# crstnbr/detqmc

Hardware: AMD Instinct MI355X
Metric: DQMC sweeps/sec (SDW-O2 L=16 beta=10 fp64) (higher is better)
Workload: dtype f64; 1 GPU; DetSDW O(2) L=16 beta=10 dtau=0.1 s=10 checkerboard delayed(32) sweepThermalization, 512 independent chains per GPU (1 process x 4 kernel contexts x 128 lockstep chains), stabilisation=qr; n_g=512, m=100, replicas_per_gpu=512, processes_per_gpu=1, contexts_per_process=4, chains_per_context=128, launch=self

## Files before the change

detqmc_amd/csrc/dqmc_context.hip:

```cpp
#include "dqmc_ctx.h"
#include <cmath>
#include <complex>
#include <cstddef>
#include <cstdio>
#include <cstdlib>
#include <cstring>
#include <string>
#include <vector>

void build_tournament(int nblk, std::vector<int>& out);

thread_local std::string g_err;

template<class T>
static int dalloc(dqmc_ctx* c, T** p, size_t count) {
    const size_t bytes = (count * sizeof(T) + 255) & ~(size_t)255;
    *p = (T*)(uintptr_t)(c->arena_off + 256);
    c->fixups.push_back((void**)p);
    c->arena_off += bytes;
    return 0;
}
static int arena_commit(dqmc_ctx* c) {
    const size_t cs = c->arena_off;
    void* q = nullptr;
// ... 242 lines not shown
            for (int y = 0; y < L; ++y)
                for (int x = 0; x < L; ++x) {
                    const int coord = dirn == 0 ? x : y;
                    if ((coord & 1) != parity) continue;
                    const int a = y * L + x, b = neigh[(dirn == 0 ? 0 : 2) * N + a];
                    M[(size_t)a * N + b] += shv; M[(size_t)b * N + a] += shv;
                }
            return M;
        };
        auto mul = [&](const std::vector<double>& A, const std::vector<double>& B) {
            std::vector<double> C((size_t)N * N, 0.0);
            for (int i = 0; i < N; ++i) for (int k = 0; k < N; ++k) { const double a = A[(size_t)i * N + k]; if (a != 0.0) for (int j = 0; j < N; ++j) C[(size_t)i * N + j] += a * B[(size_t)k * N + j]; }
            return C;
        };
        const std::vector<double> F = mul(mul(bond_matrix(0, 0, sh), bond_matrix(0, 1, sh)), mul(bond_matrix(1, 0, sh), bond_matrix(1, 1, sh)));
        const std::vector<double> Fi = mul(mul(bond_matrix(1, 1, -sh), bond_matrix(1, 0, -sh)), mul(bond_matrix(0, 1, -sh), bond_matrix(0, 0, -sh)));
        Em.assign((size_t)N * N, hc(0.0)); Ep.assign((size_t)N * N, hc(0.0));
        for (size_t i = 0; i < (size_t)N * N; ++i) { Em[i] = F[i]; Ep[i] = Fi[i]; }
    }
    out_minus.assign((size_t)ng * ng, hc(0.0)); out_plus.assign((size_t)ng * ng, hc(0.0));
    for (int b = 0; b < 2; ++b)
        for (int i = 0; i < N; ++i) for (int j = 0; j < N; ++j) {
            out_minus[(size_t)(b * N + j) * ng + (b * N + i)] = Em[(size_t)i * N + j];
            out_plus[(size_t)(b * N + j) * ng + (b * N + i)] = Ep[(size_t)i * N + j];
        }
}

static int alloc_qr_work(dqmc_ctx* c) {
    const int ng = c->n_g, np = (ng + 15) / 16;
    const size_t n2 = (size_t)ng * ng;
    int rc;
#define A_(x) if ((rc = (x))) return rc;
    A_(dalloc(c, &c->qw.V, n2)); A_(dalloc(c, &c->qw.T, (size_t)np * 2 * 256));
    A_(dalloc(c, &c->qw.W, (size_t)16 * ng)); A_(dalloc(c, &c->qw.W2, (size_t)16 * ng)); A_(dalloc(c, &c->qw.Rneg, (size_t)32 * ng));
    if (ng > 1024) { c->qw.part_count = (size_t)ng * 64 * 8; A_(dalloc(c, &c->qw.part, c->qw.part_count)); }
    A_(dalloc(c, &c->qr_perm, (size_t)ng)); A_(dalloc(c, &c->lu_swaps, (size_t)LU_SWAP_INTS)); A_(dalloc(c, &c->lu_tneg, (size_t)ng * 32)); A_(dalloc(c, &c->qr_perm_inv, (size_t)ng)); A_(dalloc(c, &c->qr_dinv, (size_t)ng));
    A_(dalloc(c, &c->rmax_inv, (size_t)ng)); A_(dalloc(c, &c->rmin, (size_t)ng));
    A_(dalloc(c, &c->lmax_inv, (size_t)ng)); A_(dalloc(c, &c->lmin, (size_t)ng));
#undef A_
    return 0;
}

static int alloc_slot(dqmc_ctx* c, UdVSlot& sl) {
    size_t n2 = (size_t)c->n_g * c->n_g;
    int rc;
    if ((rc = dalloc(c, &sl.U, n2))) return rc;
    if ((rc = dalloc(c, &sl.d, (size_t)c->n_g))) return rc;
    if ((rc = dalloc(c, &sl.Vt, n2))) return rc;
    return 0;
}

extern "C" int dqmc_create(const dqmc_params* p, dqmc_ctx** out) { return dqmc_create_batch(p, 1, out); }
static int create_fill(dqmc_ctx* c, const dqmc_params* p);

extern "C" int dqmc_create_batch(const dqmc_params* p, int nchains, dqmc_ctx** out) {
    if (!p || !out) return fail(DQMC_EINVAL, "null argument");
    *out = nullptr;
    if (nchains < 1 || nchains > 1024) return fail(DQMC_EINVAL, "nchains must be in 1..1024");
    if (p->opdim < 1 || p->opdim > 3) return fail(DQMC_EINVAL, "opdim must be 1, 2 or 3");
    if (p->L < 2 || (p->L % 2) != 0)
        return fail(DQMC_EINVAL, "Checker board decomposition only supported for even linear lattice sizes");
    if (p->weakZflux && p->opdim != 2) return fail(DQMC_EINVAL, "Magnetic field currently only supported for opdim=2");
    if (p->m < 2 || p->s < 1 || p->s >= p->m) return fail(DQMC_EINVAL, "need 0 < s < m");
    const int N = p->L * p->L, MSF = p->opdim == 3 ? 4 : 2;
    if (p->delaySteps < 1 || p->delaySteps > N) return fail(DQMC_EINVAL, "delaySteps must be in 1..N");
    if (MSF * p->delaySteps > DQMC_MAX_WDIM) return fail(DQMC_EINVAL, "MSF*delaySteps must be <= 64 on this build");
// ... 1405 lines not shown
```

detqmc_amd/csrc/dqmc_internal.h:

```cpp
#pragma once
#include <hip/hip_runtime.h>
#include <stdint.h>
#include "../../include/dqmc_hip.h"

#include <stdlib.h>
#include <float.h>
static inline const char* dev_knob(const char* name) {
#ifdef DQMC_DEV_KNOBS
    return getenv(name);
#else
    (void)name;
    return nullptr;
#endif
}

typedef double2 cplx;

#define DQMC_MAX_MSF 4
#define DQMC_MAX_WDIM 64
#define DQMC_DECIDE_WIDE_MAX_CHAINS 32

enum { SUBFAM_LU_UPDATE = 0, SUBFAM_FACT_GEMM = 1, SUBFAM_COUNT = 4 };
struct SubProf { void (*begin)(void* user, int sub); void (*end)(void* user, int sub, double flops, double bytes); void* user; };
struct Launch { hipStream_t st; int nb; size_t cs; const SubProf* sub = nullptr; };
// ... 247 lines not shown
size_t measure_custom_bond_table_cplx(int count, int N);
void launch_td_custom_onebody(const Launch& lc, const DevModel& hm, int count, const cplx* M, const unsigned* mask, const cplx* gs, cplx* ob, int t,
                              const CustomBond* bond = nullptr);
void launch_measure_td_custom(const Launch& lc, const DevModel& hm, int count, const cplx* M, const unsigned* mask, const cplx* gs, const cplx* hs,
                              const cplx* ob, double* acc, size_t acs, int row, int rows, const CustomBond* bond = nullptr);
void launch_measure_eq_custom(const Launch& lc, const DevModel& hm, int count, const cplx* M, const unsigned* mask, const cplx* M2, const unsigned* mask2,
                              const cplx* gs, cplx* ob, double* acc, const CustomBond* bond = nullptr);
struct CustomPair { const cplx* tab; const unsigned* mk; unsigned parts[DQMC_CUSTOM_MAX]; };
size_t measure_custom_pair_table_cplx(int count, int N);
void launch_measure_custom_pair(const Launch& lc, const DevModel& hm, int count, const cplx* Fa, const unsigned* mask, const cplx* gs, double* acc,
                                size_t acs, int row, int rows, const CustomPair* pair = nullptr);
size_t measure_green_matrix_row_doubles(int opdim, int N);
void launch_measure_green_matrix(const Launch& lc, const DevModel& hm, const cplx* gs, double* acc, size_t acs, int row, int rows, int apbx, int apby);
void launch_series_green_sample(const Launch& lc, const DevModel& hm, const double* fine, size_t chain_bytes, double* sample, size_t S, size_t off,
                                double* bad);
size_t series_pair_bubble_lds_bytes(int opdim, int N);
bool launch_series_pair_vertex(const Launch& lc, const DevModel& hm, const double* bins, const double* mean, const double* trig, size_t S, int B,
                               int nfreq, size_t off_chi, size_t off_g, int count, const CustomPair& pair, int qx, int qy, int apbx, int apby,
                               double* pb, double* value, double* err);
size_t series_ph_bubble_lds_bytes(int opdim, int N);
bool launch_series_ph_vertex(const Launch& lc, const DevModel& hm, const double* bins, const double* mean, const double* trig, size_t S, int B,
                             int nfreq, size_t off_chi, size_t off_g, int count, const CustomBond& bond, int qx, int qy, int apbx, int apby,
                             double* pb, double* value, double* err);
struct GreenCheckFold { double* table; size_t table_stride; int row; const double* d; const double* sv; };
size_t green_diff_partial_doubles(int n);
void launch_green_keep(const Launch& lc, const cplx* G, cplx* keep, size_t keep_stride, size_t count);
void launch_green_diff(const Launch& lc, const cplx* Gw, size_t gw_stride, const cplx* Gf, int n, int ld, int N, double* part,
                       size_t part_stride, double* out, size_t out_stride, const GreenCheckFold* fold = nullptr);
size_t measure_custom_row_doubles(int count, int N);
size_t measure_td_custom_onebody_cplx(int count, int N);
size_t measure_eq_custom_onebody_cplx(int count, int N);

struct SvdProfHooks;
struct QrWork { cplx* V; cplx* T; cplx* W; cplx* W2; cplx* Rneg; const SvdProfHooks* apply_hooks; cplx* part; size_t part_count; int* err; };
int run_qr(const Launch& lc, int n, cplx* A, cplx* Q, const QrWork& w);
int run_qr_apply_q(const Launch& lc, int n, cplx* C, const QrWork& w, int trans);
int run_qr_bgs(const Launch& lc, int n, cplx* A, cplx* Q, const QrWork& w);
void qr_reset_workspace(const Launch& lc, int n, const QrWork& w);
int run_trsm_right_upper(const Launch& lc, int n, const cplx* R, cplx* C, const QrWork& w, int trans = 0, int unit = 0,
                         const ColSrc* src = nullptr);
#define LU_SWAP_INTS 128
int run_lu(const Launch& lc, int n, cplx* A, int* perm, int* swaps, cplx* tneg);
void launch_gather_scale_cols(const Launch& lc, const cplx* X, const double* cs, const int* perm, int n, cplx* Y);
void launch_udt_init(const Launch& lc, const cplx* M, int ldm, const double* cs, const double* rs, const int* perm,
                     int transpose, cplx* W, int n);
void launch_udt_diag(const Launch& lc, const cplx* R, int n, double* d);
void launch_udt_lazy(const Launch& lc, const double* d, const int* perm, int n, double* dinv, int* perm_inv);
void launch_udt_tmat(const Launch& lc, const cplx* R, const double* d, const int* perm, int n, cplx* Tt);
void launch_permute_scale_cols(const Launch& lc, const cplx* X, const double* cs, const int* perm, int n, cplx* Y);
void launch_split_scales(const Launch& lc, const double* d, int n, double* dmax_inv, double* dmin);
void launch_logdet_vector(const Launch& lc, const cplx* R, const double* a, const double* b, int n, double* sv);
void launch_scaled_norms_rank(const Launch& lc, const cplx* M, int ldm, const double* cs, const double* rs, int transpose,
                              int n, double* norms, int* rank, double* scratch_d);
```

detqmc_amd/csrc/kernels_qr.hip:

```cpp
#include "dqmc_internal.h"
#include <cstring>

#define QR_NB 16

template<int CTRL, int ROWMASK>
__device__ __forceinline__ double q_dpp_add(double v) {
    int lo = __double2loint(v), hi = __double2hiint(v);
    int lo2 = __builtin_amdgcn_update_dpp(0, lo, CTRL, ROWMASK, 0xf, false);
    int hi2 = __builtin_amdgcn_update_dpp(0, hi, CTRL, ROWMASK, 0xf, false);
    return v + __hiloint2double(hi2, lo2);
}
__device__ __forceinline__ double q_readlane_d(double x, int l) {
    int lo = __builtin_amdgcn_readlane(__double2loint(x), l);
    int hi = __builtin_amdgcn_readlane(__double2hiint(x), l);
    return __hiloint2double(hi, lo);
}
__device__ __forceinline__ double q_wave_total(double v) {
    v = q_dpp_add<0xB1, 0xf>(v);
    v = q_dpp_add<0x4E, 0xf>(v);
    v = q_dpp_add<0x114, 0xf>(v);
    v = q_dpp_add<0x118, 0xf>(v);
    v = q_dpp_add<0x142, 0xa>(v);
    v = q_dpp_add<0x143, 0xc>(v);
    return q_readlane_d(v, 63);
}

template<int H, int MASK>
__device__ __forceinline__ void q_butterfly_level(double (&val)[32], int lane) {
    const bool hi = (lane & MASK) != 0;
#pragma unroll
    for (int j = 0; j < H; ++j) {
        double keep = hi ? val[j + H] : val[j];
        double send = hi ? val[j] : val[j + H];
        val[j] = keep + __shfl_xor(send, MASK, 64);
    }
}
// ... 112 lines not shown
                    cplx t = q_cmul(tv, w[c]);
                    a[r][c].x -= t.x;
                    a[r][c].y -= t.y;
                }
            }
        }
        if (tid < QR_NB) {
            int i = tid;
            cplx t = make_double2(0.0, 0.0);
            if (i < C) {
                cplx acc = make_double2(0.0, 0.0);
#pragma unroll
                for (int k = 0; k < QR_NB; ++k) {
                    if (k < C && k >= i) {
                        cplx tik = sT[k * QR_NB + i];
                        cplx t2 = q_cmul(tik, w[k]);
                        acc.x += t2.x; acc.y += t2.y;
                    }
                }
                cplx t3 = q_cmul(tau, acc);
                t = make_double2(-t3.x, -t3.y);
            } else if (i == C) {
                t = tau;
            }
            sT[C * QR_NB + i] = t;
            if (i == C) { sTau[C] = tau; sBeta[C] = beta; }
        }
        __syncthreads();
    }
};

template<int RPT, int NT>
__global__ __launch_bounds__(NT) void k_qr_panel(cplx* __restrict__ A, int lda, int n, int j0,
                                                  cplx* __restrict__ Vp, cplx* __restrict__ Tp, cplx* __restrict__ Tn, size_t cs) {
    __shared__ double red[2][NT / 64][2 * QR_NB];
    CHAIN(A); CHAIN(Vp); CHAIN(Tp); CHAIN(Tn);
    __shared__ cplx sT[QR_NB * QR_NB];
    __shared__ cplx sTau[QR_NB];
    __shared__ double sBeta[QR_NB];
    __shared__ cplx sAlpha;
    QrPanelState<RPT, NT> s;
    s.red = red; s.sT = sT; s.sTau = sTau; s.sBeta = sBeta; s.sAlpha = &sAlpha;
    s.tid = threadIdx.x; s.lane = threadIdx.x & 63; s.wave = threadIdx.x >> 6;
    s.rows = n - j0;
    s.ncols = (n - j0 < QR_NB) ? (n - j0) : QR_NB;
    for (int i = threadIdx.x; i < QR_NB * QR_NB; i += NT) sT[i] = make_double2(0.0, 0.0);
#pragma unroll
    for (int r = 0; r < RPT; ++r) {
        int row = s.tid + r * NT;
#pragma unroll
        for (int c = 0; c < QR_NB; ++c) {
            const cplx t = A[(size_t)(j0 + min(c, s.ncols - 1)) * lda + (j0 + min(row, s.rows - 1))];
            s.a[r][c] = (row < s.rows && c < s.ncols) ? t : make_double2(0.0, 0.0);
        }
    }
    __syncthreads();
    QrPanelStep<0>::run(s);
#pragma unroll
    for (int r = 0; r < RPT; ++r) {
        int row = s.tid + r * NT;
        if (row < s.rows) {
#pragma unroll
            for (int c = 0; c < QR_NB; ++c) {
                if (c >= s.ncols) continue;
                size_t off = (size_t)(j0 + c) * lda + (j0 + row);
                cplx x = s.a[r][c];
                if (row < c) {
                    A[off] = x;
                    Vp[off] = make_double2(0.0, 0.0);
                } else if (row == c) {
                    A[off] = make_double2(sBeta[c], 0.0);
                    Vp[off] = make_double2(1.0, 0.0);
                } else {
                    A[off] = make_double2(0.0, 0.0);
                    Vp[off] = x;
                }
            }
        }
    }
    for (int i = threadIdx.x; i < QR_NB * QR_NB; i += NT) {
        cplx t = sT[i];
        Tp[i] = t;
        Tn[i] = make_double2(-t.x, -t.y);
    }
}


typedef double q_v4d __attribute__((ext_vector_type(4)));
template<bool TRANS_T>
__global__ __launch_bounds__(256, 2) void k_qr_apply(const cplx* __restrict__ Vp, int ldv, const cplx* __restrict__ Tn,
                                                   cplx* __restrict__ C, int ldc, int rows, int ncols, int nb, size_t cs) {
    __shared__ cplx sV[64][QR_NB + 1];
    __shared__ cplx sC[64][QR_NB + 1];
    __shared__ cplx sW[QR_NB][QR_NB + 1];
    __shared__ cplx sT[QR_NB][QR_NB + 1];
    __shared__ cplx sPart[4][QR_NB][QR_NB + 1];
    CHAIN(Vp); CHAIN(Tn); CHAIN(C);
    const int tid = threadIdx.x, lane = tid & 63, wave = tid >> 6;
    const int l15 = lane & 15, l4 = lane >> 4;
    const int c0 = blockIdx.x * QR_NB;
    const int nc = min(QR_NB, ncols - c0);
    {
        int i = tid & 15, k = tid >> 4;
        sT[i][k] = (i < nb && k < nb) ? Tn[k * QR_NB + i] : make_double2(0.0, 0.0);
    }
    q_v4d w_re = (q_v4d)(0.0), w_im = (q_v4d)(0.0);
    for (int r0 = 0; r0 < rows; r0 += 64) {
        __syncthreads();
        for (int idx = tid; idx < 64 * QR_NB; idx += 256) {
            int rr = idx & 63, cc = idx >> 6;
            int row = r0 + rr;
// ... 40 lines not shown
#pragma unroll
    for (int ks = 0; ks < 4; ++ks) w2[ks] = sW[ks * 4 + l4][l15];
    for (int row0 = wave * 16; row0 < rows; row0 += 64) {
        const int row = row0 + l15;
        const bool rok = row < rows;
        cplx vf[4], cv[4];
#pragma unroll
        for (int ks = 0; ks < 4; ++ks) {
            const int k = ks * 4 + l4;
            const cplx tv = Vp[(size_t)min(k, nb - 1) * ldv + min(row, rows - 1)];
            vf[ks] = (rok && k < nb) ? tv : make_double2(0.0, 0.0);
        }
#pragma unroll
        for (int r = 0; r < 4; ++r) {
            const int j = l4 + 4 * r;
            cv[r] = C[(size_t)(c0 + min(j, nc - 1)) * ldc + min(row, rows - 1)];
        }
        q_v4d d_re = (q_v4d)(0.0), d_im = (q_v4d)(0.0);
#pragma unroll
        for (int ks = 0; ks < 4; ++ks) {
            d_re = __builtin_amdgcn_mfma_f64_16x16x4f64(w2[ks].x, vf[ks].x, d_re, 0, 0, 0);
            d_re = __builtin_amdgcn_mfma_f64_16x16x4f64(-w2[ks].y, vf[ks].y, d_re, 0, 0, 0);
            d_im = __builtin_amdgcn_mfma_f64_16x16x4f64(w2[ks].x, vf[ks].y, d_im, 0, 0, 0);
            d_im = __builtin_amdgcn_mfma_f64_16x16x4f64(w2[ks].y, vf[ks].x, d_im, 0, 0, 0);
        }
#pragma unroll
        for (int r = 0; r < 4; ++r) {
            const int j = l4 + 4 * r;
            if (rok && j < nc) C[(size_t)(c0 + j) * ldc + row] = make_double2(cv[r].x + d_re[r], cv[r].y + d_im[r]);
        }
    }
}

#define QR_MAXREF 4
#define QR_FENCE() do { asm volatile("" ::: "memory"); __builtin_amdgcn_sched_barrier(0); } while (0)
#define QR_TIE(acc, ptr) asm volatile("" : "+v"(acc), "+v"(ptr))
struct QrRefs { const cplx* V[QR_MAXREF]; const cplx* Tn[QR_MAXREF]; int nb[QR_MAXREF]; int n; };
template<bool TRANS_T, int NCH>
__global__ __launch_bounds__(256, 2) void k_qr_apply_reg(QrRefs refs, int ldv, cplx* __restrict__ C, int ldc, int rows, int ncols, size_t cs, int nb_chains) {
    __shared__ cplx sW[QR_NB][QR_NB + 1];
    __shared__ cplx sT[QR_NB][QR_NB + 1];
    __shared__ cplx sPart[4][QR_NB][QR_NB + 1];
    int chain, cblk;
    xcd_chain_tile((ncols + QR_NB - 1) / QR_NB, nb_chains, chain, cblk);
    C = chain_ptr_i(C, cs, chain);
    constexpr int RW = 16 * NCH;
    constexpr int NE = 4 * NCH;
    const int tid = threadIdx.x, lane = tid & 63, wave = tid >> 6;
    const int l15 = lane & 15, l4 = lane >> 4;
    const int c0 = cblk * QR_NB;
    const int nc = min(QR_NB, ncols - c0);
    const int slab = wave * RW;
    const int rlast = rows - 1;
    const bool cok = l15 < nc;
    cplx* Ccol = C + (size_t)(c0 + (cok ? l15 : 0)) * ldc;
    cplx creg[NE];
#pragma unroll
    for (int e = 0; e < NE; ++e) {
        const int row = slab + 4 * e + l4;
        const cplx t = nt_load(Ccol + min(row, rlast));
        creg[e] = (cok && row < rows) ? t : make_double2(0.0, 0.0);
    }
    const int wi = tid & 15, wj = tid >> 4;
    for (int rf = 0; rf < refs.n; ++rf) {
#if defined(__HIP_DEVICE_COMPILE__)
        typedef const cplx __attribute__((address_space(1)))* gcplx;
#else
        typedef const cplx* gcplx;
#endif
        gcplx Vp = (gcplx)chain_ptr_i(refs.V[rf], cs, chain);
        gcplx Tn = (gcplx)chain_ptr_i(refs.Tn[rf], cs, chain);
        const int nb = refs.nb[rf];
        int rl = rlast, rw = rows;
        asm volatile("" : "+v"(rl), "+s"(rw));
        __syncthreads();
        {
            const cplx t = Tn[wj * QR_NB + wi];
            sT[wi][wj] = (wi < nb && wj < nb) ? t : make_double2(0.0, 0.0);
        }
        const bool vok = l15 < nb;
        gcplx Vcol = Vp + (size_t)(vok ? l15 : 0) * ldv;
        q_v4d w_re = (q_v4d)(0.0), w_im = (q_v4d)(0.0), w_p2 = (q_v4d)(0.0);
        constexpr int CH = 4;
        cplx va[CH], vb[CH];
        auto loadv = [&](gcplx base, int e0, cplx (&dst)[CH]) {
            int rb = slab + l4;
            asm volatile("" : "+v"(rb));
#pragma unroll
            for (int i = 0; i < CH; ++i) {
                if (e0 + i >= NE) continue;
                const int row = rb + 4 * (e0 + i);
                dst[i] = base[min(row, rl)];
            }
        };
        auto mac = [&](int e0, const cplx (&src)[CH]) {
#pragma unroll
            for (int i = 0; i < CH; ++i) {
                if (e0 + i >= NE) continue;
                const cplx v = src[i];
                const cplx x = creg[e0 + i];
                w_re = __builtin_amdgcn_mfma_f64_16x16x4f64(v.x, x.x, w_re, 0, 0, 0);
                w_p2 = __builtin_amdgcn_mfma_f64_16x16x4f64(-v.y, x.y, w_p2, 0, 0, 0);
                w_im = __builtin_amdgcn_mfma_f64_16x16x4f64(v.x - v.y, x.x + x.y, w_im, 0, 0, 0);
            }
        };
        gcplx vbase = Vcol;
        loadv(vbase, 0, va);
        if (CH < NE) loadv(vbase, CH, vb);
        __builtin_amdgcn_sched_barrier(0);
#pragma unroll
        for (int c = 0; c < NE; c += 2 * CH) {
            mac(c, va);
            __builtin_amdgcn_sched_barrier(0);
            if (c + 2 * CH < NE) { QR_TIE(w_re, vbase); loadv(vbase, c + 2 * CH, va); __builtin_amdgcn_sched_barrier(0); }
            if (c + CH < NE) { mac(c + CH, vb); __builtin_amdgcn_sched_barrier(0); }
            if (c + 3 * CH < NE) { QR_TIE(w_re, vbase); loadv(vbase, c + 3 * CH, vb); __builtin_amdgcn_sched_barrier(0); }
        }
#pragma unroll
        for (int r = 0; r < 4; ++r) sPart[wave][l4 + 4 * r][l15] = make_double2(w_re[r] - w_p2[r], (w_im[r] - w_re[r]) - w_p2[r]);
        __syncthreads();
        {
            cplx p0 = sPart[0][wi][wj], p1 = sPart[1][wi][wj], p2 = sPart[2][wi][wj], p3 = sPart[3][wi][wj];
            sW[wi][wj] = make_double2((p0.x + p1.x) + (p2.x + p3.x), (p0.y + p1.y) + (p2.y + p3.y));
        }
        __syncthreads();
        {
            cplx a2 = make_double2(0.0, 0.0);
#pragma unroll
            for (int k = 0; k < QR_NB; ++k) {
                cplx t = TRANS_T ? make_double2(sT[k][wi].x, -sT[k][wi].y) : sT[wi][k];
                cplx w = sW[k][wj];
                a2.x += t.x * w.x - t.y * w.y;
                a2.y += t.x * w.y + t.y * w.x;
            }
            __syncthreads();
            sW[wi][wj] = a2;
        }
        __syncthreads();
        cplx w2[4];
#pragma unroll
        for (int ks = 0; ks < 4; ++ks) w2[ks] = sW[ks * 4 + l4][l15];
        cplx vfa[4], vfb[4];
        auto loadvf = [&](gcplx base, int t, cplx (&dst)[4]) {
            const int vrow = slab + 16 * t + l15;
            const int vr = min(vrow, rl);
#pragma unroll
            for (int ks = 0; ks < 4; ++ks) {
                const int k = ks * 4 + l4;
                dst[ks] = base[(size_t)min(k, nb - 1) * ldv + vr];
            }
        };
        double w2s[4];
#pragma unroll
        for (int ks = 0; ks < 4; ++ks) w2s[ks] = w2[ks].x + w2[ks].y;
        q_v4d d_re, d_im, d_p2;
        auto upd = [&](int t, const cplx (&vf)[4]) {
            d_re = (q_v4d)(0.0); d_im = (q_v4d)(0.0); d_p2 = (q_v4d)(0.0);
#pragma unroll
            for (int ks = 0; ks < 4; ++ks) {
                d_re = __builtin_amdgcn_mfma_f64_16x16x4f64(vf[ks].x, w2[ks].x, d_re, 0, 0, 0);
                d_p2 = __builtin_amdgcn_mfma_f64_16x16x4f64(vf[ks].y, w2[ks].y, d_p2, 0, 0, 0);
                d_im = __builtin_amdgcn_mfma_f64_16x16x4f64(vf[ks].x + vf[ks].y, w2s[ks], d_im, 0, 0, 0);
            }
        };
        auto put = [&](int t) {
            int rb = slab + l4;
            asm volatile("" : "+v"(rb));
#pragma unroll
            for (int r = 0; r < 4; ++r) {
                const bool rin = rb + 16 * t + 4 * r < rw;
                creg[4 * t + r].x = rin ? creg[4 * t + r].x + (d_re[r] - d_p2[r]) : 0.0;
                creg[4 * t + r].y = rin ? creg[4 * t + r].y + ((d_im[r] - d_re[r]) - d_p2[r]) : 0.0;
            }
        };
        gcplx pbase = Vp;
        loadvf(pbase, 0, vfa);
        if (NCH > 1) loadvf(pbase, 1, vfb);
        __builtin_amdgcn_sched_barrier(0);
#pragma unroll
        for (int t = 0; t < NCH; t += 2) {
            upd(t, vfa);
            __builtin_amdgcn_sched_barrier(0);
            if (t + 2 < NCH) { QR_TIE(d_re, pbase); loadvf(pbase, t + 2, vfa); __builtin_amdgcn_sched_barrier(0); }
            put(t);
            if (t + 1 < NCH) {
                upd(t + 1, vfb);
                __builtin_amdgcn_sched_barrier(0);
                if (t + 3 < NCH) { QR_TIE(d_re, pbase); loadvf(pbase, t + 3, vfb); __builtin_amdgcn_sched_barrier(0); }
                put(t + 1);
            }
        }
    }
#pragma unroll
    for (int e = 0; e < NE; ++e) {
        const int row = slab + 4 * e + l4;
        if (cok && row < rows) nt_store(Ccol + row, creg[e]);
    }
}

template<bool TRANS_T>
static void launch_apply_reg(const Launch& lc, dim3 grid, const QrRefs& r, int ldv, cplx* C, int ldc, int rows, int ncols) {
    if (lc.nb % 8 == 0) grid = dim3(grid.x * lc.nb, 1, 1);
    switch ((rows + 63) / 64) {
        case 1: hipLaunchKernelGGL((k_qr_apply_reg<TRANS_T, 1>), grid, dim3(256), 0, lc.st, r, ldv, C, ldc, rows, ncols, lc.cs, lc.nb); break;
        case 2: hipLaunchKernelGGL((k_qr_apply_reg<TRANS_T, 2>), grid, dim3(256), 0, lc.st, r, ldv, C, ldc, rows, ncols, lc.cs, lc.nb); break;
        case 3: hipLaunchKernelGGL((k_qr_apply_reg<TRANS_T, 3>), grid, dim3(256), 0, lc.st, r, ldv, C, ldc, rows, ncols, lc.cs, lc.nb); break;
        case 4: hipLaunchKernelGGL((k_qr_apply_reg<TRANS_T, 4>), grid, dim3(256), 0, lc.st, r, ldv, C, ldc, rows, ncols, lc.cs, lc.nb); break;
        case 5: hipLaunchKernelGGL((k_qr_apply_reg<TRANS_T, 5>), grid, dim3(256), 0, lc.st, r, ldv, C, ldc, rows, ncols, lc.cs, lc.nb); break;
        case 6: hipLaunchKernelGGL((k_qr_apply_reg<TRANS_T, 6>), grid, dim3(256), 0, lc.st, r, ldv, C, ldc, rows, ncols, lc.cs, lc.nb); break;
        case 7: hipLaunchKernelGGL((k_qr_apply_reg<TRANS_T, 7>), grid, dim3(256), 0, lc.st, r, ldv, C, ldc, rows, ncols, lc.cs, lc.nb); break;
        default: hipLaunchKernelGGL((k_qr_apply_reg<TRANS_T, 8>), grid, dim3(256), 0, lc.st, r, ldv, C, ldc, rows, ncols, lc.cs, lc.nb); break;
    }
}

static void gemm_small(const Launch& lc, int opA, int opB, const cplx* A, int lda, const cplx* B, int ldb, cplx* C, int ldc,
                       int M, int N, int K, int accumulate) {
    GemmArgs g = GemmArgs();
    g.A = A; g.lda = lda; g.opA = opA; g.B = B; g.ldb = ldb; g.opB = opB; g.C = C; g.ldc = ldc;
    g.M = M; g.N = N; g.K = K; g.Kmul = 1; g.accumulate = accumulate;
    launch_gemm(lc, g);
}

static void launch_panel(const Launch& lc, cplx* A, int n, int j0, cplx* V, cplx* Tp, cplx* Tn) {
    const int rows = n - j0;
    if (rows > 2560) {
        if (rows <= 3072) hipLaunchKernelGGL((k_qr_panel<3, 1024>), dim3(1, 1, lc.nb), dim3(1024), 0, lc.st, A, n, n, j0, V, Tp, Tn, lc.cs);
        else              hipLaunchKernelGGL((k_qr_panel<4, 1024>), dim3(1, 1, lc.nb), dim3(1024), 0, lc.st, A, n, n, j0, V, Tp, Tn, lc.cs);
        return;
    }
    if (rows > 1024) {
        switch ((rows + 511) / 512) {
            case 3: hipLaunchKernelGGL((k_qr_panel<3, 512>), dim3(1, 1, lc.nb), dim3(512), 0, lc.st, A, n, n, j0, V, Tp, Tn, lc.cs); break;
            case 4: hipLaunchKernelGGL((k_qr_panel<4, 512>), dim3(1, 1, lc.nb), dim3(512), 0, lc.st, A, n, n, j0, V, Tp, Tn, lc.cs); break;
            default: hipLaunchKernelGGL((k_qr_panel<5, 512>), dim3(1, 1, lc.nb), dim3(512), 0, lc.st, A, n, n, j0, V, Tp, Tn, lc.cs); break;
        }
        return;
    }
    const int rpt = (rows + 255) / 256;
    switch (rpt) {
        case 1: hipLaunchKernelGGL((k_qr_panel<1, 256>), dim3(1, 1, lc.nb), dim3(256), 0, lc.st, A, n, n, j0, V, Tp, Tn, lc.cs); break;
        case 2: hipLaunchKernelGGL((k_qr_panel<2, 256>), dim3(1, 1, lc.nb), dim3(256), 0, lc.st, A, n, n, j0, V, Tp, Tn, lc.cs); break;
        case 3: hipLaunchKernelGGL((k_qr_panel<3, 256>), dim3(1, 1, lc.nb), dim3(256), 0, lc.st, A, n, n, j0, V, Tp, Tn, lc.cs); break;
        case 4: hipLaunchKernelGGL((k_qr_panel<4, 256>), dim3(1, 1, lc.nb), dim3(256), 0, lc.st, A, n, n, j0, V, Tp, Tn, lc.cs); break;
        default: break;
    }
}

int run_qr(const Launch& lc, int n, cplx* A, cplx* Q, const QrWork& w) {
    int launches = 0;
    const int np = (n + QR_NB - 1) / QR_NB;
    const bool reg = n <= 512;
    auto Tneg = [&](int p) { return w.T + (size_t)p * 2 * QR_NB * QR_NB + QR_NB * QR_NB; };
    auto Vat = [&](int pcol, int prow) { return w.V + (size_t)(pcol * QR_NB) * n + prow * QR_NB; };
    auto nbof = [&](int p) { return (n - p * QR_NB < QR_NB) ? (n - p * QR_NB) : QR_NB; };
    auto apply = [&](bool transT, cplx* M, int rb, int col0, int ncols, int p0, int step, int count) {
        const int rows = n - rb * QR_NB;
        cplx* C = M + (size_t)col0 * n + rb * QR_NB;
        const dim3 grid((ncols + QR_NB - 1) / QR_NB, 1, lc.nb);
        if (w.apply_hooks) w.apply_hooks->begin(w.apply_hooks->user);
        if (reg) {
            QrRefs r;
            r.n = count;
            for (int i = 0; i < QR_MAXREF; ++i) { r.V[i] = nullptr; r.Tn[i] = nullptr; r.nb[i] = 0; }
            for (int i = 0; i < count; ++i) { const int p = p0 + i * step; r.V[i] = Vat(p, rb); r.Tn[i] = Tneg(p); r.nb[i] = nbof(p); }
            if (transT) launch_apply_reg<true>(lc, grid, r, n, C, n, rows, ncols);
            else        launch_apply_reg<false>(lc, grid, r, n, C, n, rows, ncols);
        } else {
            if (transT) hipLaunchKernelGGL((k_qr_apply<true>), grid, dim3(256), 0, lc.st, Vat(p0, rb), n, Tneg(p0), C, n, rows, ncols, nbof(p0), lc.cs);
            else        hipLaunchKernelGGL((k_qr_apply<false>), grid, dim3(256), 0, lc.st, Vat(p0, rb), n, Tneg(p0), C, n, rows, ncols, nbof(p0), lc.cs);
        }
        if (w.apply_hooks) w.apply_hooks->end(w.apply_hooks->user, 1);
        ++launches;
    };
    auto panel = [&](int p) {
        cplx* Tp = w.T + (size_t)p * 2 * QR_NB * QR_NB;
        launch_panel(lc, A, n, p * QR_NB, w.V, Tp, Tp + QR_NB * QR_NB);
        ++launches;
    };
    for (int p = 0; p < np;) {
        const int j0 = p * QR_NB;
        const int left = n - j0;
        if (reg && left > 4 * QR_NB) {
            panel(p);
            apply(true, A, p, j0 + QR_NB, QR_NB, p, 1, 1);
            panel(p + 1);
            apply(true, A, p, j0 + 2 * QR_NB, 2 * QR_NB, p, 1, 2);
            panel(p + 2);
            apply(true, A, p + 2, j0 + 3 * QR_NB, QR_NB, p + 2, 1, 1);
            panel(p + 3);
            apply(true, A, p, j0 + 4 * QR_NB, left - 4 * QR_NB, p, 1, 4);
            p += 4;
        } else if (reg && left > 2 * QR_NB) {
            panel(p);
            apply(true, A, p, j0 + QR_NB, QR_NB, p, 1, 1);
            panel(p + 1);
            apply(true, A, p, j0 + 2 * QR_NB, left - 2 * QR_NB, p, 1, 2);
            p += 2;
        } else {
            panel(p);
            const int ntrail = left - nbof(p);
            if (ntrail > 0) apply(true, A, p, j0 + nbof(p), ntrail, p, 1, 1);
            p += 1;
        }
    }
    if (!Q) return launches;
    launch_set_identity(lc, Q, n);
    ++launches;
    for (int p = np - 1; p >= 0;) {
        int cnt = 1;
        if (reg && nbof(p) == QR_NB) cnt = (p >= 3) ? 4 : (p >= 1 ? 2 : 1);
        const int lo = p - (cnt - 1);
        apply(false, Q, lo, lo * QR_NB, n - lo * QR_NB, p, -1, cnt);
        p -= cnt;
    }
    return launches;
}

int run_qr_apply_q(const Launch& lc, int n, cplx* C, const QrWork& w, int trans) {
    int launches = 0;
    const int np = (n + QR_NB - 1) / QR_NB;
    const bool reg = n <= 512;
    auto nbof = [&](int p) { return (n - p * QR_NB < QR_NB) ? (n - p * QR_NB) : QR_NB; };
    auto group = [&](int first, int step, int cnt, int lo) {
        const int rows = n - lo * QR_NB;
        cplx* Cs = C + lo * QR_NB;
        const dim3 grid((n + QR_NB - 1) / QR_NB, 1, lc.nb);
        if (w.apply_hooks) w.apply_hooks->begin(w.apply_hooks->user);
        if (reg) {
            QrRefs r;
            r.n = cnt;
            for (int i = 0; i < QR_MAXREF; ++i) { r.V[i] = nullptr; r.Tn[i] = nullptr; r.nb[i] = 0; }
            for (int i = 0; i < cnt; ++i) {
                const int q = first + i * step;
                r.V[i] = w.V + (size_t)(q * QR_NB) * n + lo * QR_NB;
                r.Tn[i] = w.T + (size_t)q * 2 * QR_NB * QR_NB + QR_NB * QR_NB;
                r.nb[i] = nbof(q);
            }
            if (trans) launch_apply_reg<true>(lc, grid, r, n, Cs, n, rows, n);
            else       launch_apply_reg<false>(lc, grid, r, n, Cs, n, rows, n);
        } else {
            const cplx* Vq = w.V + (size_t)(first * QR_NB) * n + lo * QR_NB;
            const cplx* Tq = w.T + (size_t)first * 2 * QR_NB * QR_NB + QR_NB * QR_NB;
            if (trans) hipLaunchKernelGGL((k_qr_apply<true>), grid, dim3(256), 0, lc.st, Vq, n, Tq, Cs, n, rows, n, nbof(first), lc.cs);
            else       hipLaunchKernelGGL((k_qr_apply<false>), grid, dim3(256), 0, lc.st, Vq, n, Tq, Cs, n, rows, n, nbof(first), lc.cs);
        }
        if (w.apply_hooks) w.apply_hooks->end(w.apply_hooks->user, 1);
        ++launches;
    };
    if (trans) {
        for (int p = 0; p < np;) {
            int cnt = 1;
            if (reg) { cnt = (np - p >= 4) ? 4 : ((np - p >= 2) ? 2 : 1); if (nbof(p + cnt - 1) != QR_NB) cnt = 1; }
            group(p, 1, cnt, p);
            p += cnt;
        }
    } else {
        for (int p = np - 1; p >= 0;) {
            int cnt = 1;
            if (reg && nbof(p) == QR_NB) cnt = (p >= 3) ? 4 : (p >= 1 ? 2 : 1);
            group(p, -1, cnt, p - (cnt - 1));
            p -= cnt;
        }
    }
    return launches;
}

#define TRSM_NB 32
__global__ __launch_bounds__(256) void k_trsm_block(cplx* __restrict__ C, int ldc, const cplx* __restrict__ R, int ldr,
                                                     int n, int j0, int nb, int trans, int unit, size_t cs, ColSrc S) {
    __shared__ cplx sR[TRSM_NB][TRSM_NB + 1];
    CHAIN(C); CHAIN(R); CHAIN(S.X); CHAIN(S.idx); CHAIN(S.scale);
    for (int i = threadIdx.x; i < TRSM_NB * TRSM_NB; i += 256) {
// ... 325 lines not shown
```

Baseline: 300.9 sweeps/s.

## Add full-tile QR apply path with row-major compact V copy

Adds a specialised mode to the register-blocked QR reflector apply kernel. When rows, columns and leading dimensions are tile-aligned, it drops bounds checks and clamping on C and V loads and stores. The panel kernel also writes a row-major, zero-padded copy of each Householder block (VR), so the first-stage V loads become contiguous. This trades extra panel writes and workspace for cheaper, coalesced inner-loop loads, and adds more kernel instantiations.

```diff
diff --git a/detqmc_amd/csrc/dqmc_context.hip b/detqmc_amd/csrc/dqmc_context.hip
--- a/detqmc_amd/csrc/dqmc_context.hip
+++ b/detqmc_amd/csrc/dqmc_context.hip
@@ -298,6 +298,7 @@
     int rc;
 #define A_(x) if ((rc = (x))) return rc;
     A_(dalloc(c, &c->qw.V, n2)); A_(dalloc(c, &c->qw.T, (size_t)np * 2 * 256));
+    if (ng <= 512) A_(dalloc(c, &c->qw.VR, (size_t)np * 16 * ng));
     A_(dalloc(c, &c->qw.W, (size_t)16 * ng)); A_(dalloc(c, &c->qw.W2, (size_t)16 * ng)); A_(dalloc(c, &c->qw.Rneg, (size_t)32 * ng));
     if (ng > 1024) { c->qw.part_count = (size_t)ng * 64 * 8; A_(dalloc(c, &c->qw.part, c->qw.part_count)); }
     A_(dalloc(c, &c->qr_perm, (size_t)ng)); A_(dalloc(c, &c->lu_swaps, (size_t)LU_SWAP_INTS)); A_(dalloc(c, &c->lu_tneg, (size_t)ng * 32)); A_(dalloc(c, &c->qr_perm_inv, (size_t)ng)); A_(dalloc(c, &c->qr_dinv, (size_t)ng));
diff --git a/detqmc_amd/csrc/dqmc_internal.h b/detqmc_amd/csrc/dqmc_internal.h
--- a/detqmc_amd/csrc/dqmc_internal.h
+++ b/detqmc_amd/csrc/dqmc_internal.h
@@ -303,7 +303,8 @@
 size_t measure_eq_custom_onebody_cplx(int count, int N);
 
 struct SvdProfHooks;
-struct QrWork { cplx* V; cplx* T; cplx* W; cplx* W2; cplx* Rneg; const SvdProfHooks* apply_hooks; cplx* part; size_t part_count; int* err; };
+struct QrWork { cplx* V; cplx* T; cplx* W; cplx* W2; cplx* Rneg; const SvdProfHooks* apply_hooks; cplx* part; size_t part_count; int* err;
+                cplx* VR; int apply_path; int* apply_full; };
 int run_qr(const Launch& lc, int n, cplx* A, cplx* Q, const QrWork& w);
 int run_qr_apply_q(const Launch& lc, int n, cplx* C, const QrWork& w, int trans);
 int run_qr_bgs(const Launch& lc, int n, cplx* A, cplx* Q, const QrWork& w);
diff --git a/detqmc_amd/csrc/kernels_qr.hip b/detqmc_amd/csrc/kernels_qr.hip
--- a/detqmc_amd/csrc/kernels_qr.hip
+++ b/detqmc_amd/csrc/kernels_qr.hip
@@ -2,6 +2,7 @@
 #include <cstring>
 
 #define QR_NB 16
+#define QR_MAXREF 4
 
 template<int CTRL, int ROWMASK>
 __device__ __forceinline__ double q_dpp_add(double v) {
@@ -180,9 +181,9 @@
 
 template<int RPT, int NT>
 __global__ __launch_bounds__(NT) void k_qr_panel(cplx* __restrict__ A, int lda, int n, int j0,
-                                                  cplx* __restrict__ Vp, cplx* __restrict__ Tp, cplx* __restrict__ Tn, size_t cs) {
+                                                  cplx* __restrict__ Vp, cplx* __restrict__ Tp, cplx* __restrict__ Tn, cplx* __restrict__ VRp, size_t cs) {
     __shared__ double red[2][NT / 64][2 * QR_NB];
-    CHAIN(A); CHAIN(Vp); CHAIN(Tp); CHAIN(Tn);
+    CHAIN(A); CHAIN(Vp); CHAIN(Tp); CHAIN(Tn); CHAIN(VRp);
     __shared__ cplx sT[QR_NB * QR_NB];
     __shared__ cplx sTau[QR_NB];
     __shared__ double sBeta[QR_NB];
@@ -224,7 +225,19 @@
                     Vp[off] = x;
                 }
             }
-        }
+            if (VRp) {
+                cplx* vr = VRp + (size_t)(j0 + row) * QR_NB;
+#pragma unroll
+                for (int c = 0; c < QR_NB; ++c) {
+                    const cplx x = s.a[r][c];
+                    vr[c] = (row < c || c >= s.ncols) ? make_double2(0.0, 0.0) : (row == c ? make_double2(1.0, 0.0) : x);
+                }
+            }
+        }
+    }
+    if (VRp) {
+        const int nz = min(j0, (QR_MAXREF - 1) * QR_NB);
+        for (int i = threadIdx.x; i < nz * QR_NB; i += NT) VRp[(size_t)(j0 - nz) * QR_NB + i] = make_double2(0.0, 0.0);
     }
     for (int i = threadIdx.x; i < QR_NB * QR_NB; i += NT) {
         cplx t = sT[i];
@@ -331,12 +344,15 @@
     }
 }
 
-#define QR_MAXREF 4
 #define QR_FENCE() do { asm volatile("" ::: "memory"); __builtin_amdgcn_sched_barrier(0); } while (0)
 #define QR_TIE(acc, ptr) asm volatile("" : "+v"(acc), "+v"(ptr))
-struct QrRefs { const cplx* V[QR_MAXREF]; const cplx* Tn[QR_MAXREF]; int nb[QR_MAXREF]; int n; };
-template<bool TRANS_T, int NCH>
+struct QrRefs { const cplx* V[QR_MAXREF]; const cplx* Tn[QR_MAXREF]; const cplx* VR[QR_MAXREF]; int nb[QR_MAXREF]; int n; };
+#define QR_GENERIC 0
+#define QR_FULL 1
+#define QR_FULL_VR 2
+template<bool TRANS_T, int NCH, int MODE>
 __global__ __launch_bounds__(256, 2) void k_qr_apply_reg(QrRefs refs, int ldv, cplx* __restrict__ C, int ldc, int rows, int ncols, size_t cs, int nb_chains) {
+    constexpr bool FULL = MODE != QR_GENERIC;
     __shared__ cplx sW[QR_NB][QR_NB + 1];
     __shared__ cplx sT[QR_NB][QR_NB + 1];
     __shared__ cplx sPart[4][QR_NB][QR_NB + 1];
@@ -353,9 +369,12 @@
     const int rlast = rows - 1;
     const bool cok = l15 < nc;
     cplx* Ccol = C + (size_t)(c0 + (cok ? l15 : 0)) * ldc;
+    cplx* const Cblk = C + (size_t)c0 * ldc;
+    const unsigned coff = (unsigned)l15 * (unsigned)ldc + (unsigned)(slab + l4);
     cplx creg[NE];
 #pragma unroll
     for (int e = 0; e < NE; ++e) {
+        if (FULL) { creg[e] = nt_load(&(Cblk + 4 * e)[coff]); continue; }
         const int row = slab + 4 * e + l4;
         const cplx t = nt_load(Ccol + min(row, rlast));
         creg[e] = (cok && row < rows) ? t : make_double2(0.0, 0.0);
@@ -375,14 +394,22 @@
         __syncthreads();
         {
             const cplx t = Tn[wj * QR_NB + wi];
-            sT[wi][wj] = (wi < nb && wj < nb) ? t : make_double2(0.0, 0.0);
+            sT[wi][wj] = (FULL || (wi < nb && wj < nb)) ? t : make_double2(0.0, 0.0);
         }
         const bool vok = l15 < nb;
         gcplx Vcol = Vp + (size_t)(vok ? l15 : 0) * ldv;
+        gcplx v1base = MODE == QR_FULL_VR ? (gcplx)chain_ptr_i(refs.VR[rf], cs, chain) : Vp;
+        constexpr int V1STEP = MODE == QR_FULL_VR ? 4 * QR_NB : 4;
+        unsigned v1off = MODE == QR_FULL_VR ? (unsigned)(slab + l4) * QR_NB + (unsigned)l15 : (unsigned)l15 * (unsigned)ldv + (unsigned)(slab + l4);
         q_v4d w_re = (q_v4d)(0.0), w_im = (q_v4d)(0.0), w_p2 = (q_v4d)(0.0);
         constexpr int CH = 4;
         cplx va[CH], vb[CH];
         auto loadv = [&](gcplx base, int e0, cplx (&dst)[CH]) {
+            if (FULL) {
+#pragma unroll
+                for (int i = 0; i < CH; ++i) dst[i] = (v1base + V1STEP * (e0 + i))[v1off];
+                return;
+            }
             int rb = slab + l4;
             asm volatile("" : "+v"(rb));
 #pragma unroll
@@ -411,9 +438,9 @@
         for (int c = 0; c < NE; c += 2 * CH) {
             mac(c, va);
             __builtin_amdgcn_sched_barrier(0);
-            if (c + 2 * CH < NE) { QR_TIE(w_re, vbase); loadv(vbase, c + 2 * CH, va); __builtin_amdgcn_sched_barrier(0); }
+            if (c + 2 * CH < NE) { if (FULL) QR_TIE(w_re, v1off); else QR_TIE(w_re, vbase); loadv(vbase, c + 2 * CH, va); __builtin_amdgcn_sched_barrier(0); }
             if (c + CH < NE) { mac(c + CH, vb); __builtin_amdgcn_sched_barrier(0); }
-            if (c + 3 * CH < NE) { QR_TIE(w_re, vbase); loadv(vbase, c + 3 * CH, vb); __builtin_amdgcn_sched_barrier(0); }
+            if (c + 3 * CH < NE) { if (FULL) QR_TIE(w_re, v1off); else QR_TIE(w_re, vbase); loadv(vbase, c + 3 * CH, vb); __builtin_amdgcn_sched_barrier(0); }
         }
 #pragma unroll
         for (int r = 0; r < 4; ++r) sPart[wave][l4 + 4 * r][l15] = make_double2(w_re[r] - w_p2[r], (w_im[r] - w_re[r]) - w_p2[r]);
@@ -440,7 +467,13 @@
 #pragma unroll
         for (int ks = 0; ks < 4; ++ks) w2[ks] = sW[ks * 4 + l4][l15];
         cplx vfa[4], vfb[4];
+        unsigned v2off = (unsigned)l4 * (unsigned)ldv + (unsigned)(slab + l15);
         auto loadvf = [&](gcplx base, int t, cplx (&dst)[4]) {
+            if (FULL) {
+#pragma unroll
+                for (int ks = 0; ks < 4; ++ks) dst[ks] = (Vp + ((size_t)(4 * ks) * ldv + 16 * t))[v2off];
+                return;
+            }
             const int vrow = slab + 16 * t + l15;
             const int vr = min(vrow, rl);
 #pragma unroll
@@ -463,6 +496,14 @@
             }
         };
         auto put = [&](int t) {
+            if (FULL) {
+#pragma unroll
+                for (int r = 0; r < 4; ++r) {
+                    creg[4 * t + r].x = creg[4 * t + r].x + (d_re[r] - d_p2[r]);
+                    creg[4 * t + r].y = creg[4 * t + r].y + ((d_im[r] - d_re[r]) - d_p2[r]);
+                }
+                return;
+            }
             int rb = slab + l4;
             asm volatile("" : "+v"(rb));
 #pragma unroll
@@ -480,36 +521,49 @@
         for (int t = 0; t < NCH; t += 2) {
             upd(t, vfa);
             __builtin_amdgcn_sched_barrier(0);
-            if (t + 2 < NCH) { QR_TIE(d_re, pbase); loadvf(pbase, t + 2, vfa); __builtin_amdgcn_sched_barrier(0); }
+            if (t + 2 < NCH) { if (FULL) QR_TIE(d_re, v2off); else QR_TIE(d_re, pbase); loadvf(pbase, t + 2, vfa); __builtin_amdgcn_sched_barrier(0); }
             put(t);
             if (t + 1 < NCH) {
                 upd(t + 1, vfb);
                 __builtin_amdgcn_sched_barrier(0);
-                if (t + 3 < NCH) { QR_TIE(d_re, pbase); loadvf(pbase, t + 3, vfb); __builtin_amdgcn_sched_barrier(0); }
+                if (t + 3 < NCH) { if (FULL) QR_TIE(d_re, v2off); else QR_TIE(d_re, pbase); loadvf(pbase, t + 3, vfb); __builtin_amdgcn_sched_barrier(0); }
                 put(t + 1);
             }
         }
     }
 #pragma unroll
     for (int e = 0; e < NE; ++e) {
+        if (FULL) { nt_store(&(Cblk + 4 * e)[coff], creg[e]); continue; }
         const int row = slab + 4 * e + l4;
         if (cok && row < rows) nt_store(Ccol + row, creg[e]);
     }
 }
 
+template<bool TRANS_T, int MODE>
+static void launch_apply_reg_mode(const Launch& lc, dim3 grid, const QrRefs& r, int ldv, cplx* C, int ldc, int rows, int ncols) {
+    switch ((rows + 63) / 64) {
+        case 1: hipLaunchKernelGGL((k_qr_apply_reg<TRANS_T, 1, MODE>), grid, dim3(256), 0, lc.st, r, ldv, C, ldc, rows, ncols, lc.cs, lc.nb); break;
+        case 2: hipLaunchKernelGGL((k_qr_apply_reg<TRANS_T, 2, MODE>), grid, dim3(256), 0, lc.st, r, ldv, C, ldc, rows, ncols, lc.cs, lc.nb); break;
+        case 3: hipLaunchKernelGGL((k_qr_apply_reg<TRANS_T, 3, MODE>), grid, dim3(256), 0, lc.st, r, ldv, C, ldc, rows, ncols, lc.cs, lc.nb); break;
+        case 4: hipLaunchKernelGGL((k_qr_apply_reg<TRANS_T, 4, MODE>), grid, dim3(256), 0, lc.st, r, ldv, C, ldc, rows, ncols, lc.cs, lc.nb); break;
+        case 5: hipLaunchKernelGGL((k_qr_apply_reg<TRANS_T, 5, MODE>), grid, dim3(256), 0, lc.st, r, ldv, C, ldc, rows, ncols, lc.cs, lc.nb); break;
+        case 6: hipLaunchKernelGGL((k_qr_apply_reg<TRANS_T, 6, MODE>), grid, dim3(256), 0, lc.st, r, ldv, C, ldc, rows, ncols, lc.cs, lc.nb); break;
+        case 7: hipLaunchKernelGGL((k_qr_apply_reg<TRANS_T, 7, MODE>), grid, dim3(256), 0, lc.st, r, ldv, C, ldc, rows, ncols, lc.cs, lc.nb); break;
+        default: hipLaunchKernelGGL((k_qr_apply_reg<TRANS_T, 8, MODE>), grid, dim3(256), 0, lc.st, r, ldv, C, ldc, rows, ncols, lc.cs, lc.nb); break;
+    }
+}
 template<bool TRANS_T>
-static void launch_apply_reg(const Launch& lc, dim3 grid, const QrRefs& r, int ldv, cplx* C, int ldc, int rows, int ncols) {
+static int launch_apply_reg(const Launch& lc, dim3 grid, const QrRefs& r, int ldv, cplx* C, int ldc, int rows, int ncols, int path) {
+    static const bool knob_full = !(dev_knob("DQMC_QR_FULL") && atoi(dev_knob("DQMC_QR_FULL")) == 0);
+    static const bool knob_vr = !(dev_knob("DQMC_QR_VR") && atoi(dev_knob("DQMC_QR_VR")) == 0);
     if (lc.nb % 8 == 0) grid = dim3(grid.x * lc.nb, 1, 1);
-    switch ((rows + 63) / 64) {
-        case 1: hipLaunchKernelGGL((k_qr_apply_reg<TRANS_T, 1>), grid, dim3(256), 0, lc.st, r, ldv, C, ldc, rows, ncols, lc.cs, lc.nb); break;
-        case 2: hipLaunchKernelGGL((k_qr_apply_reg<TRANS_T, 2>), grid, dim3(256), 0, lc.st, r, ldv, C, ldc, rows, ncols, lc.cs, lc.nb); break;
-        case 3: hipLaunchKernelGGL((k_qr_apply_reg<TRANS_T, 3>), grid, dim3(256), 0, lc.st, r, ldv, C, ldc, rows, ncols, lc.cs, lc.nb); break;
-        case 4: hipLaunchKernelGGL((k_qr_apply_reg<TRANS_T, 4>), grid, dim3(256), 0, lc.st, r, ldv, C, ldc, rows, ncols, lc.cs, lc.nb); break;
-        case 5: hipLaunchKernelGGL((k_qr_apply_reg<TRANS_T, 5>), grid, dim3(256), 0, lc.st, r, ldv, C, ldc, rows, ncols, lc.cs, lc.nb); break;
-        case 6: hipLaunchKernelGGL((k_qr_apply_reg<TRANS_T, 6>), grid, dim3(256), 0, lc.st, r, ldv, C, ldc, rows, ncols, lc.cs, lc.nb); break;
-        case 7: hipLaunchKernelGGL((k_qr_apply_reg<TRANS_T, 7>), grid, dim3(256), 0, lc.st, r, ldv, C, ldc, rows, ncols, lc.cs, lc.nb); break;
-        default: hipLaunchKernelGGL((k_qr_apply_reg<TRANS_T, 8>), grid, dim3(256), 0, lc.st, r, ldv, C, ldc, rows, ncols, lc.cs, lc.nb); break;
-    }
+    bool full = path != 1 && (path == 2 || knob_full) && rows % 64 == 0 && ncols % QR_NB == 0 && ldv % 64 == 0 && ldc % 64 == 0;
+    bool vr = path == 2 || knob_vr;
+    for (int i = 0; i < r.n; ++i) { full = full && r.nb[i] == QR_NB; vr = vr && r.VR[i] != nullptr; }
+    if (!full) launch_apply_reg_mode<TRANS_T, QR_GENERIC>(lc, grid, r, ldv, C, ldc, rows, ncols);
+    else if (vr) launch_apply_reg_mode<TRANS_T, QR_FULL_VR>(lc, grid, r, ldv, C, ldc, rows, ncols);
+    else launch_apply_reg_mode<TRANS_T, QR_FULL>(lc, grid, r, ldv, C, ldc, rows, ncols);
+    return full ? 1 : 0;
 }
 
 static void gemm_small(const Launch& lc, int opA, int opB, const cplx* A, int lda, const cplx* B, int ldb, cplx* C, int ldc,
@@ -520,27 +574,27 @@
     launch_gemm(lc, g);
 }
 
-static void launch_panel(const Launch& lc, cplx* A, int n, int j0, cplx* V, cplx* Tp, cplx* Tn) {
+static void launch_panel(const Launch& lc, cplx* A, int n, int j0, cplx* V, cplx* Tp, cplx* Tn, cplx* VRp) {
     const int rows = n - j0;
     if (rows > 2560) {
-        if (rows <= 3072) hipLaunchKernelGGL((k_qr_panel<3, 1024>), dim3(1, 1, lc.nb), dim3(1024), 0, lc.st, A, n, n, j0, V, Tp, Tn, lc.cs);
-        else              hipLaunchKernelGGL((k_qr_panel<4, 1024>), dim3(1, 1, lc.nb), dim3(1024), 0, lc.st, A, n, n, j0, V, Tp, Tn, lc.cs);
+        if (rows <= 3072) hipLaunchKernelGGL((k_qr_panel<3, 1024>), dim3(1, 1, lc.nb), dim3(1024), 0, lc.st, A, n, n, j0, V, Tp, Tn, VRp, lc.cs);
+        else              hipLaunchKernelGGL((k_qr_panel<4, 1024>), dim3(1, 1, lc.nb), dim3(1024), 0, lc.st, A, n, n, j0, V, Tp, Tn, VRp, lc.cs);
         return;
     }
     if (rows > 1024) {
         switch ((rows + 511) / 512) {
-            case 3: hipLaunchKernelGGL((k_qr_panel<3, 512>), dim3(1, 1, lc.nb), dim3(512), 0, lc.st, A, n, n, j0, V, Tp, Tn, lc.cs); break;
-            case 4: hipLaunchKernelGGL((k_qr_panel<4, 512>), dim3(1, 1, lc.nb), dim3(512), 0, lc.st, A, n, n, j0, V, Tp, Tn, lc.cs); break;
-            default: hipLaunchKernelGGL((k_qr_panel<5, 512>), dim3(1, 1, lc.nb), dim3(512), 0, lc.st, A, n, n, j0, V, Tp, Tn, lc.cs); break;
+            case 3: hipLaunchKernelGGL((k_qr_panel<3, 512>), dim3(1, 1, lc.nb), dim3(512), 0, lc.st, A, n, n, j0, V, Tp, Tn, VRp, lc.cs); break;
+            case 4: hipLaunchKernelGGL((k_qr_panel<4, 512>), dim3(1, 1, lc.nb), dim3(512), 0, lc.st, A, n, n, j0, V, Tp, Tn, VRp, lc.cs); break;
+            default: hipLaunchKernelGGL((k_qr_panel<5, 512>), dim3(1, 1, lc.nb), dim3(512), 0, lc.st, A, n, n, j0, V, Tp, Tn, VRp, lc.cs); break;
         }
         return;
     }
     const int rpt = (rows + 255) / 256;
     switch (rpt) {
-        case 1: hipLaunchKernelGGL((k_qr_panel<1, 256>), dim3(1, 1, lc.nb), dim3(256), 0, lc.st, A, n, n, j0, V, Tp, Tn, lc.cs); break;
-        case 2: hipLaunchKernelGGL((k_qr_panel<2, 256>), dim3(1, 1, lc.nb), dim3(256), 0, lc.st, A, n, n, j0, V, Tp, Tn, lc.cs); break;
-        case 3: hipLaunchKernelGGL((k_qr_panel<3, 256>), dim3(1, 1, lc.nb), dim3(256), 0, lc.st, A, n, n, j0, V, Tp, Tn, lc.cs); break;
-        case 4: hipLaunchKernelGGL((k_qr_panel<4, 256>), dim3(1, 1, lc.nb), dim3(256), 0, lc.st, A, n, n, j0, V, Tp, Tn, lc.cs); break;
+        case 1: hipLaunchKernelGGL((k_qr_panel<1, 256>), dim3(1, 1, lc.nb), dim3(256), 0, lc.st, A, n, n, j0, V, Tp, Tn, VRp, lc.cs); break;
+        case 2: hipLaunchKernelGGL((k_qr_panel<2, 256>), dim3(1, 1, lc.nb), dim3(256), 0, lc.st, A, n, n, j0, V, Tp, Tn, VRp, lc.cs); break;
+        case 3: hipLaunchKernelGGL((k_qr_panel<3, 256>), dim3(1, 1, lc.nb), dim3(256), 0, lc.st, A, n, n, j0, V, Tp, Tn, VRp, lc.cs); break;
+        case 4: hipLaunchKernelGGL((k_qr_panel<4, 256>), dim3(1, 1, lc.nb), dim3(256), 0, lc.st, A, n, n, j0, V, Tp, Tn, VRp, lc.cs); break;
         default: break;
     }
 }
@@ -552,6 +606,7 @@
     auto Tneg = [&](int p) { return w.T + (size_t)p * 2 * QR_NB * QR_NB + QR_NB * QR_NB; };
     auto Vat = [&](int pcol, int prow) { return w.V + (size_t)(pcol * QR_NB) * n + prow * QR_NB; };
     auto nbof = [&](int p) { return (n - p * QR_NB < QR_NB) ? (n - p * QR_NB) : QR_NB; };
+    auto VRat = [&](int pcol, int prow) { return w.VR ? w.VR + (size_t)pcol * QR_NB * n + (size_t)prow * QR_NB * QR_NB : nullptr; };
     auto apply = [&](bool transT, cplx* M, int rb, int col0, int ncols, int p0, int step, int count) {
         const int rows = n - rb * QR_NB;
         cplx* C = M + (size_t)col0 * n + rb * QR_NB;
@@ -560,10 +615,11 @@
         if (reg) {
             QrRefs r;
             r.n = count;
-            for (int i = 0; i < QR_MAXREF; ++i) { r.V[i] = nullptr; r.Tn[i] = nullptr; r.nb[i] = 0; }
-            for (int i = 0; i < count; ++i) { const int p = p0 + i * step; r.V[i] = Vat(p, rb); r.Tn[i] = Tneg(p); r.nb[i] = nbof(p); }
-            if (transT) launch_apply_reg<true>(lc, grid, r, n, C, n, rows, ncols);
-            else        launch_apply_reg<false>(lc, grid, r, n, C, n, rows, ncols);
+            for (int i = 0; i < QR_MAXREF; ++i) { r.V[i] = nullptr; r.Tn[i] = nullptr; r.VR[i] = nullptr; r.nb[i] = 0; }
+            for (int i = 0; i < count; ++i) { const int p = p0 + i * step; r.V[i] = Vat(p, rb); r.Tn[i] = Tneg(p); r.VR[i] = VRat(p, rb); r.nb[i] = nbof(p); }
+            const int full = transT ? launch_apply_reg<true>(lc, grid, r, n, C, n, rows, ncols, w.apply_path)
+                                    : launch_apply_reg<false>(lc, grid, r, n, C, n, rows, ncols, w.apply_path);
+            if (w.apply_full) *w.apply_full += full;
         } else {
             if (transT) hipLaunchKernelGGL((k_qr_apply<true>), grid, dim3(256), 0, lc.st, Vat(p0, rb), n, Tneg(p0), C, n, rows, ncols, nbof(p0), lc.cs);
             else        hipLaunchKernelGGL((k_qr_apply<false>), grid, dim3(256), 0, lc.st, Vat(p0, rb), n, Tneg(p0), C, n, rows, ncols, nbof(p0), lc.cs);
@@ -573,7 +629,7 @@
     };
     auto panel = [&](int p) {
         cplx* Tp = w.T + (size_t)p * 2 * QR_NB * QR_NB;
-        launch_panel(lc, A, n, p * QR_NB, w.V, Tp, Tp + QR_NB * QR_NB);
+        launch_panel(lc, A, n, p * QR_NB, w.V, Tp, Tp + QR_NB * QR_NB, VRat(p, 0));
         ++launches;
     };
     for (int p = 0; p < np;) {
@@ -628,15 +684,17 @@
         if (reg) {
             QrRefs r;
             r.n = cnt;
-            for (int i = 0; i < QR_MAXREF; ++i) { r.V[i] = nullptr; r.Tn[i] = nullptr; r.nb[i] = 0; }
+            for (int i = 0; i < QR_MAXREF; ++i) { r.V[i] = nullptr; r.Tn[i] = nullptr; r.VR[i] = nullptr; r.nb[i] = 0; }
             for (int i = 0; i < cnt; ++i) {
                 const int q = first + i * step;
                 r.V[i] = w.V + (size_t)(q * QR_NB) * n + lo * QR_NB;
                 r.Tn[i] = w.T + (size_t)q * 2 * QR_NB * QR_NB + QR_NB * QR_NB;
+                r.VR[i] = w.VR ? w.VR + (size_t)q * QR_NB * n + (size_t)lo * QR_NB * QR_NB : nullptr;
                 r.nb[i] = nbof(q);
             }
-            if (trans) launch_apply_reg<true>(lc, grid, r, n, Cs, n, rows, n);
-            else       launch_apply_reg<false>(lc, grid, r, n, Cs, n, rows, n);
+            const int full = trans ? launch_apply_reg<true>(lc, grid, r, n, Cs, n, rows, n, w.apply_path)
+                                   : launch_apply_reg<false>(lc, grid, r, n, Cs, n, rows, n, w.apply_path);
+            if (w.apply_full) *w.apply_full += full;
         } else {
             const cplx* Vq = w.V + (size_t)(first * QR_NB) * n + lo * QR_NB;
             const cplx* Tq = w.T + (size_t)first * 2 * QR_NB * QR_NB + QR_NB * QR_NB;
```

Result: no change. 303.4 sweeps/s (median of 6 runs) (+0.8%).
